# CESNET/GPUJPEG

Hardware: NVIDIA H100
Metric: Mpix/s encode+decode 8k RGB q75 (higher is better)
Workload: dtype f32+i32 (u8 in, i16 coefficients)

## Files before the change

gpujpeg_b200/csrc/gj_encoder.c:

```c
#include <assert.h>
#include <stdlib.h>
#include <string.h>

#include "gj_internal.h"

#define GJ_STRIPES 8
#define GJ_STRIPE_MIN_BYTES ((size_t)8 << 20)

struct gpujpeg_encoder {
    gj_stream_t stream;
    int device;
    struct gpujpeg_parameters param;
    struct gpujpeg_image_parameters param_image;
    int initialised;
    struct gj_geometry geo;
    struct gj_k1_request k1_req;
    struct gj_k1_plan k1;
    uint8_t* d_planes; size_t d_planes_size;
    struct gj_raw_layout raw;
    int quality;
    enum gpujpeg_header_type header_type;
    enum gpujpeg_header_type header_written;
    int flipped;
    unsigned channel_remap;
// ... 434 lines not shown
}

static int fit_huffman_tables(struct gpujpeg_encoder* e)
{
    const struct gj_geometry* g = &e->geo;
    if ( launch_stats(e) || gj_cuda_memcpy_d2h_async(e->h_counts, e->d_counts, GJ_HUFF_COUNTS_BYTES, e->stream) ||
         gj_cuda_stream_sync(e->stream) )
        return -1;
    int used[2] = {0, 0};
    for ( int c = 0; c < g->comp_count; c++ )
        used[g->lay.comp_tbl[c]] = 1;
    for ( int t = 0; t < 2; t++ ) {
        for ( int k = 0; k < 2; k++ ) {
            if ( used[t] ) gj_huff_spec_optimal(e->h_counts + (t * 2 + k) * 256, &e->spec[t][k]);
            else gj_huff_spec_default(t, k, &e->spec[t][k]);
        }
        gj_enc_lut_build(&e->spec[t][0], &e->spec[t][1], &e->h_tab.lut[t]);
    }
    e->spec_custom = 1;
    const size_t need = GJ_HEADER_BASE_CAP + 4 * 256 + gj_exif_tags_bytes(e->extras.exif_tags) + e->extras.com_size;
    if ( need > e->header_cap ) {
        free(e->header);
        e->header = (uint8_t*)malloc(need);
        e->header_cap = e->header ? need : 0;
        if ( !e->header ) return -1;
    }
    e->header_size = gj_write_header(e->header, &e->param, &e->param_image, e->raw_q, e->spec, e->header_type, &e->extras);
    if ( e->header_size + 64 > g->stream_cap ) {
        GJ_ERR("The header (%zu bytes) does not fit the stream buffer of a %dx%d image.\n", e->header_size, g->width, g->height);
        return -1;
    }
    return gj_cuda_memcpy_h2d_async(e->d_tab, &e->h_tab, sizeof e->h_tab, e->stream);
}

static struct gj_k1_request k1_request(const struct gpujpeg_encoder* e, int in)
{
    struct gj_k1_request r;
    memset(&r, 0, sizeof r);
    r.in = in;
    r.libjpeg = e->writer_libjpeg;
    r.flipped = e->flipped != 0;
    r.channel_remap = e->channel_remap != 0;
    r.coef_input = e->coef_input;
    return r;
}

static int reserve_out(struct gpujpeg_encoder* e, size_t size)
{
    if ( e->out_size >= size && e->out_is_pinned == e->out_pinned ) return 0;
    if ( e->out ) {
        if ( e->out_is_pinned ) gj_cuda_free_host(e->out);
        else free(e->out);
    }
    e->out = NULL;
    e->out_size = 0;
    e->out_is_pinned = e->out_pinned;
    if ( e->out_pinned ) {
        if ( gj_cuda_malloc_host((void**)&e->out, size) ) return -1;
    }
    else if ( !(e->out = (uint8_t*)malloc(size)) ) {
        return -1;
    }
    e->out_size = size;
    return 0;
}

static int encoder_init_image(struct gpujpeg_encoder* e, const struct gpujpeg_parameters* p,
                              const struct gpujpeg_image_parameters* pi, const struct gj_k1_request* k1)
{
    gj_geometry_init(&e->geo, p, pi);
    e->geo.stream_cap += e->extras.com_size;
    e->k1_req = *k1;
    gj_k1_choose(&e->geo, k1, &e->k1);
    if ( e->k1.raw_layout && gj_raw_layout_init(&e->raw, pi) ) return -1;
    if ( e->k1.convert && grow((void**)&e->d_planes, &e->d_planes_size, e->k1.planes_bytes) ) return -1;
    const struct gj_geometry* g = &e->geo;
    size_t coef_bytes = g->coef_count * sizeof(int16_t);
    const size_t segblk_all = (size_t)g->seg_mcu * (size_t)g->lay.bpm;
    size_t first_stride = (segblk_all * 48 + 2 + 127) / 128 * 128;
    if ( first_stride > g->slot_stride ) first_stride = g->slot_stride;
    if ( e->slot_stride < first_stride || e->slot_stride > g->slot_stride ) e->slot_stride = first_stride;
    size_t tmp_bytes = (size_t)g->seg_count * e->slot_stride + 256;
    const int segblk = g->seg_mcu * g->lay.bpm;
    size_t spill_bytes = (size_t)g->seg_count * (segblk <= 40 ? segblk : 32) * 32 * sizeof(uint32_t);
    const size_t split_bytes = gj_huffman_split_status_bytes(g->seg_count, segblk, g->slot_stride);
    if ( grow((void**)&e->d_coef, &e->d_coef_size, coef_bytes) ||
         grow((void**)&e->d_nzmask, &e->d_nzmask_size, g->coef_count / 64 * sizeof(uint64_t)) ||
         grow((void**)&e->d_tmp, &e->d_tmp_size, tmp_bytes) ||
         grow((void**)&e->d_spill, &e->d_spill_size, spill_bytes) ||
         grow((void**)&e->d_split, &e->d_split_size, split_bytes) ||
         grow((void**)&e->d_stream, &e->d_stream_size, g->stream_cap + 64) ) {
        GJ_ERR("Encoder device allocation failed (%zu + %zu + %zu bytes): %s\n", coef_bytes, tmp_bytes, g->stream_cap,
               gj_cuda_last_error());
        return -1;
    }
    if ( g->seg_count > e->seg_alloc ) {
        gj_cuda_free(e->d_seg_bytes);
        gj_cuda_free(e->d_seg_off);
        e->d_seg_bytes = NULL;
        e->d_seg_off = NULL;
        e->seg_alloc = 0;
        if ( gj_cuda_malloc((void**)&e->d_seg_bytes, (size_t)g->seg_count * 4) ||
             gj_cuda_malloc((void**)&e->d_seg_off, (size_t)g->seg_count * 8) )
            return -1;
        e->seg_alloc = g->seg_count;
    }
    if ( reserve_out(e, g->stream_cap) ) return -1;
    e->param = *p;
    e->param_image = *pi;
    e->initialised = 1;
    return 0;
}

static int same_image(const struct gpujpeg_image_parameters* a, const struct gpujpeg_image_parameters* b)
{
    return a->width == b->width && a->height == b->height && a->color_space == b->color_space &&
           a->pixel_format == b->pixel_format && a->width_padding == b->width_padding;
}
static gpujpeg_sampling_factor_t packed_sampling(const struct gpujpeg_parameters* p)
{
    gpujpeg_sampling_factor_t r = 0;
    for ( int c = 0; c < p->comp_count && c < 4; c++ )
        r |= (gpujpeg_sampling_factor_t)p->sampling_factor[c].horizontal << (28 - 8 * c) |
             (gpujpeg_sampling_factor_t)p->sampling_factor[c].vertical << (24 - 8 * c);
    return r;
}

static int same_param(const struct gpujpeg_parameters* a, const struct gpujpeg_parameters* b)
{
    if ( a->restart_interval != b->restart_interval || a->interleaved != b->interleaved ||
         a->segment_info != b->segment_info || a->comp_count != b->comp_count ||
         a->color_space_internal != b->color_space_internal )
        return 0;
    for ( int c = 0; c < a->comp_count; c++ )
        if ( a->sampling_factor[c].horizontal != b->sampling_factor[c].horizontal ||
             a->sampling_factor[c].vertical != b->sampling_factor[c].vertical )
            return 0;
    return 1;
}

static struct gpujpeg_parameters adjust_params(struct gpujpeg_encoder* e, const struct gpujpeg_parameters* param,
                                               const struct gpujpeg_image_parameters* pi, int img_changed)
{
    struct gpujpeg_parameters a = *param;
    if ( param->comp_count == 0 ) {
        if ( img_changed || !e->initialised ) {
            const int n = gpujpeg_pixel_format_get_comp_count(pi->pixel_format);
            a.comp_count = n > 3 ? 3 : n;
            struct gj_raw_layout rl;
            const int known = gj_raw_layout_init(&rl, pi) == 0;
            memset(a.sampling_factor, 0, sizeof a.sampling_factor);
            for ( int c = 0; c < a.comp_count; c++ ) {
                a.sampling_factor[c].horizontal = known ? rl.sampling[c].horizontal : 1;
                a.sampling_factor[c].vertical = known ? rl.sampling[c].vertical : 1;
            }
        }
        else {
            a.comp_count = e->param.comp_count;
            memcpy(a.sampling_factor, e->param.sampling_factor, sizeof a.sampling_factor);
        }
    }
    if ( param->restart_interval == RESTART_AUTO ) {
        if ( img_changed || !e->initialised || a.interleaved != e->param.interleaved )
            a.restart_interval =
                gpujpeg_encoder_suggest_restart_interval(pi, packed_sampling(&a), a.interleaved, a.verbose);
        else
            a.restart_interval = e->param.restart_interval;
// ... 582 lines not shown
```

gpujpeg_b200/csrc/gj_huffman.cu:

```cuda
#include <cuda_runtime.h>
#include <stdint.h>

#include "gj_device.cuh"
#include "gj_internal.h"
#include "gj_launch.cuh"

namespace {

constexpr unsigned FULL = 0xFFFFFFFFu;

__device__ __forceinline__ int warp_incl_scan(int v, int lane)
{
#pragma unroll
    for ( int d = 1; d < 32; d <<= 1 ) {
        const int t = __shfl_up_sync(FULL, v, d);
        if ( lane >= d ) v += t;
    }
    return v;
}

__device__ __forceinline__ int scan_of_segment(const gj_scan_layout& L, int g)
{
    return (g >= L.scan_seg_begin[1]) + (g >= L.scan_seg_begin[2]) + (g >= L.scan_seg_begin[3]);
}

__device__ __forceinline__ void segment_block(const gj_scan_layout& L, int scan, int first_mcu, int j, size_t& bi, int& comp,
                                              int& pd)
{
    if ( L.simple ) {
        if ( !L.interleaved ) {
            comp = scan;
            bi = (size_t)L.blk_off[scan] + first_mcu + j;
            pd = 1;
        }
        else {
            const int cps = L.comp_count;
            const int mcu = j / cps;
            comp = j - mcu * cps;
            bi = (size_t)L.blk_off[comp] + first_mcu + mcu;
            pd = cps;
        }
    }
    else if ( !L.interleaved ) {
        comp = scan;
        bi = (size_t)L.blk_off[scan] + first_mcu + j;
        pd = 1;
    }
    else {
        const int mcu = j / L.bpm, i = j - mcu * L.bpm;
        const int m = first_mcu + mcu;
        const int my = m / L.mcu_x, mx = m - my * L.mcu_x;
        comp = L.idx_comp[i];
        bi = (size_t)L.blk_off[comp] + (size_t)(my * L.comp_vs[comp] + L.idx_dy[i]) * L.bcx[comp] + mx * L.comp_hs[comp] +
             L.idx_dx[i];
        pd = L.idx_pred[i];
    }
}


constexpr int HE_WARPS = 8;
constexpr int HE_WORDS = 512;
constexpr int HE_CAP_BITS = (HE_WORDS - 2) * 32;

__device__ __forceinline__ uint32_t flush_words(const uint32_t* buf, int nw, uint8_t* out, uint32_t pos, int lane, uint32_t cap)
{
    for ( int base = 0; base < nw; base += 32 ) {
        const int i = base + lane;
        const uint32_t w = i < nw ? buf[i] : 0u;
        int cnt = 0;
        if ( i < nw ) {
            const uint32_t t = w & (w >> 4) & 0x0F0F0F0Fu;
            const uint32_t ff = t & (t >> 2) & 0x03030303u;
            const uint32_t m = ff & (ff >> 1) & 0x01010101u;
            cnt = 4 + __popc(m);
        }
        const int incl = warp_incl_scan(cnt, lane);
        uint8_t* o = out + pos + (incl - cnt);
        if ( i < nw && pos + (uint32_t)incl <= cap ) {
#pragma unroll
            for ( int j = 3; j >= 0; j-- ) {
                const uint8_t b = (uint8_t)(w >> (8 * j));
                *o++ = b;
                if ( b == 0xFF ) *o++ = 0;
            }
        }
        pos += (uint32_t)__shfl_sync(FULL, incl, 31);
    }
    return pos;
}

constexpr int HE_PRIV = 25;
constexpr int HE_SPILL = 32;
constexpr int HE_HEAD = 12;
template <class Put>
__device__ __forceinline__ int code_block(int dc, int pred, uint64_t nz, const int16_t* head16, const int16_t* __restrict__ blk,
                                          const uint32_t (*s_ac)[256], const uint32_t (*s_dc)[16], int tbl, Put put)
{
    uint64_t acc = 0;
    int nb = 0, wi = 0;
    auto emit = [&](int len, uint32_t bits) {
        acc = (acc << len) | (uint64_t)bits;
        nb += len;
        if ( nb >= 32 ) {
            put(wi, (uint32_t)(acc >> (nb - 32)));
            wi++;
            nb -= 32;
        }
    };
    const int diff = dc - pred;
    const int dcat = gj_category(diff);
    const uint32_t de = s_dc[tbl][dcat];
    emit((int)(de & 31u) + dcat, ((de >> 5) << dcat) | (dcat ? gj_value_bits(diff, dcat) : 0u));
    uint32_t mlo = (uint32_t)nz & ~1u, mhi = (uint32_t)(nz >> 32);
    int last = 0;
    const uint32_t zrl = s_ac[tbl][0xF0];
    while ( mlo | mhi ) {
        int k;
        if ( mlo ) { k = __ffs((int)mlo) - 1; mlo &= mlo - 1; }
        else { k = 32 + __ffs((int)mhi) - 1; mhi &= mhi - 1; }
        int run = k - last - 1;
        last = k;
        const int v = k < 16 ? (int)head16[k] : (int)__ldg(blk + k);
        const int size = gj_category(v);
        while ( run > 15 ) {
            emit((int)(zrl & 31u), zrl >> 5);
            run -= 16;
        }
        const uint32_t e = s_ac[tbl][(run << 4) | size];
        emit((int)(e & 31u) + size, ((e >> 5) << size) | gj_value_bits(v, size));
    }
    if ( last < 63 ) {
        const uint32_t e = s_ac[tbl][0];
        emit((int)(e & 31u), e >> 5);
    }
    if ( nb ) put(wi, (uint32_t)(acc << (32 - nb)));
    return 32 * wi + nb;
}

constexpr int HE_SMEM = (2 * 256 + 2 * 16 + HE_WARPS * HE_WORDS + HE_WARPS * 32 * HE_PRIV + HE_WARPS * 32 * HE_HEAD) * 4;

__global__ void __launch_bounds__(HE_WARPS * 32)
k_huff_encode(const int16_t* __restrict__ coef, const uint64_t* __restrict__ nzmask, const __grid_constant__ gj_scan_layout lay,
              int seg_mcu, int seg_count, uint8_t* __restrict__ tmp, size_t slot_stride,
              uint32_t* __restrict__ seg_bytes, uint32_t* __restrict__ spill_all, const gj_dev_enc_tables* __restrict__ tables,
              uint64_t* __restrict__ info, unsigned long long* __restrict__ place_status, int n_status)
{
    gj_pdl_wait();
    if ( threadIdx.x == 0 && (int)blockIdx.x < n_status ) place_status[blockIdx.x] = 0ull;
    const uint32_t slot_cap = (uint32_t)slot_stride;
    extern __shared__ __align__(16) uint32_t he_smem[];
    uint32_t (*s_ac)[256] = reinterpret_cast<uint32_t (*)[256]>(he_smem);
    uint32_t (*s_dc)[16] = reinterpret_cast<uint32_t (*)[16]>(he_smem + 512);
    uint32_t* s_buf = he_smem + 512 + 32;
    uint32_t* s_priv = s_buf + HE_WARPS * HE_WORDS;
    uint32_t* s_head = s_priv + HE_WARPS * 32 * HE_PRIV;

    for ( int i = threadIdx.x; i < 512; i += blockDim.x )
        s_ac[i >> 8][i & 255] = tables->lut[i >> 8].ac[i & 255];
    if ( threadIdx.x < 32 ) s_dc[threadIdx.x >> 4][threadIdx.x & 15] = tables->lut[threadIdx.x >> 4].dc[threadIdx.x & 15];
    __syncthreads();

    const int warp = threadIdx.x >> 5, lane = threadIdx.x & 31;
    const int g = blockIdx.x * HE_WARPS + warp;
    if ( g >= seg_count ) return;
    const int scan = scan_of_segment(lay, g), s = g - lay.scan_seg_begin[scan];
    const int first_mcu = s * seg_mcu;
    const int mcus = min(seg_mcu, lay.scan_mcus[scan] - first_mcu);
    const int nblocks = mcus * lay.bpm;
    uint32_t* buf = s_buf + warp * HE_WORDS;
    uint32_t* priv = s_priv + (warp * 32 + lane) * HE_PRIV;
    uint32_t* spill = spill_all + ((size_t)g * 32 + lane) * HE_SPILL;
    uint32_t* head = s_head + (warp * 32 + lane) * HE_HEAD;
    const int16_t* head16 = reinterpret_cast<const int16_t*>(head);
    uint8_t* out = tmp + (size_t)g * slot_stride;
    uint32_t out_pos = 0;
    int carry = 0;

    for ( int i = lane; i < HE_WORDS; i += 32 )
        buf[i] = 0;
    __syncwarp();

    int dc_before = 0;
    uint64_t nz_next = 0;
    uint4 ha_next = make_uint4(0u, 0u, 0u, 0u), hb_next = ha_next;
    size_t bi_next = 0;
    int comp_next = 0, pd_next = 1;
    {
        const int j = lane;
        if ( j < nblocks ) {
            segment_block(lay, scan, first_mcu, j, bi_next, comp_next, pd_next);
            nz_next = __ldg(nzmask + bi_next);
            ha_next = __ldg(reinterpret_cast<const uint4*>(coef + bi_next * 64));
            hb_next = __ldg(reinterpret_cast<const uint4*>(coef + bi_next * 64) + 1);
        }
    }
    for ( int base = 0; base < nblocks; base += 32 ) {
        const int j = base + lane;
        const bool active = j < nblocks;
        const int comp = comp_next, pd = pd_next;
        const int tbl = lay.comp_tbl[comp];
        const int16_t* blk = coef + bi_next * 64;

        const uint64_t nz = nz_next;
        const int dc = (int)(short)(ha_next.x & 0xFFFFu);
        reinterpret_cast<uint4*>(head)[0] = ha_next;
        reinterpret_cast<uint4*>(head)[1] = hb_next;
        nz_next = 0;
        ha_next = hb_next = make_uint4(0u, 0u, 0u, 0u);
        {
            const int jn = j + 32;
            if ( jn < nblocks ) {
                segment_block(lay, scan, first_mcu, jn, bi_next, comp_next, pd_next);
                nz_next = __ldg(nzmask + bi_next);
                ha_next = __ldg(reinterpret_cast<const uint4*>(coef + bi_next * 64));
                hb_next = __ldg(reinterpret_cast<const uint4*>(coef + bi_next * 64) + 1);
            }
        }
        const int from = (lane - pd) & 31;
        int pred = __shfl_sync(FULL, dc, from);
        const int pred_before = __shfl_sync(FULL, dc_before, from);
        if ( lane < pd ) pred = pred_before;
        if ( j < pd ) pred = 0;
        dc_before = dc;

        int len = 0;
        if ( active ) {
            len = code_block(dc, pred, nz, head16, blk, s_ac, s_dc, tbl, [&](int wi, uint32_t w) {
                if ( wi < HE_PRIV ) priv[wi] = w;
                else spill[wi - HE_PRIV] = w;
            });
        }
        const int incl = warp_incl_scan(len, lane);
        const int excl = incl - len;

        int lane0 = 0;
        while ( lane0 < 32 ) {
            const int rel0 = __shfl_sync(FULL, excl, lane0);
            const int mypos = carry + (excl - rel0);
            const bool fits = lane >= lane0 && mypos + len <= HE_CAP_BITS;
            const int nfit = __popc(__ballot_sync(FULL, fits));
            if ( nfit == 0 ) break;
            const bool mine = lane >= lane0 && lane < lane0 + nfit;
            if ( mine && len > 0 ) {
                const int nw = (len + 31) >> 5;
                const int d0 = mypos >> 5, sh = mypos & 31;
                const int endbit = mypos + len;
                uint32_t prev = 0;
                for ( int q = 0; q <= nw; q++ ) {
                    const uint32_t w = q < nw ? (q < HE_PRIV ? priv[q] : spill[q - HE_PRIV]) : 0u;
                    const uint32_t o = sh ? (prev | (w >> sh)) : w;
                    prev = sh ? (w << (32 - sh)) : 0u;
                    const int d = d0 + q;
                    if ( 32 * d >= endbit ) break;
                    if ( 32 * d >= mypos && 32 * d + 32 <= endbit ) buf[d] = o;
                    else atomicOr(&buf[d], o);
                }
            }
            __syncwarp();
            const int lastl = lane0 + nfit - 1;
            const int newbits = carry + (__shfl_sync(FULL, incl, lastl) - rel0);
            const int nwords = newbits >> 5;
            out_pos = flush_words(buf, nwords, out, out_pos, lane, slot_cap);
            __syncwarp();
            const uint32_t tail = buf[nwords];
            __syncwarp();
            for ( int i = lane; i <= nwords; i += 32 )
                buf[i] = 0;
            __syncwarp();
            if ( lane == 0 ) buf[0] = tail;
            __syncwarp();
            carry = newbits & 31;
            lane0 += nfit;
        }
    }

    if ( lane == 0 ) {
        uint32_t w = buf[0];
        const int nbytes = (carry + 7) >> 3;
        if ( carry & 7 ) w |= ((1u << (8 - (carry & 7))) - 1u) << (32 - nbytes * 8);
        uint32_t n = out_pos;
        for ( int q = 0; q < nbytes; q++ ) {
            const uint8_t b = (uint8_t)(w >> (24 - 8 * q));
            if ( n + 2u <= slot_cap ) {
                out[n] = b;
                if ( b == 0xFF ) out[n + 1] = 0;
            }
            n += b == 0xFF ? 2u : 1u;
        }
        seg_bytes[g] = n;
        if ( n + 2u > slot_cap ) {
            atomicOr(reinterpret_cast<unsigned long long*>(info + 1), 2ull);
            atomicMax(reinterpret_cast<unsigned long long*>(info + 2), (unsigned long long)n + 2ull);
        }
    }
}

constexpr int HP_MAXBLK = 40;
constexpr int HP_THREADS_MAX = HE_WARPS * HP_MAXBLK;
static_assert(HE_WARPS * HE_WORDS >= HP_THREADS_MAX * HE_HEAD, "heads must fit into the stream buffers");
constexpr int HP_SMEM = (2 * 256 + 2 * 16 + HE_WARPS * HE_WORDS + HE_WARPS * HP_MAXBLK * HE_PRIV + HE_WARPS * HP_MAXBLK) * 4;

struct SegPick {
    int n[GJ_MAX_COMP], lo[GJ_MAX_COMP];
    int total;
    int zero_status;
};
__device__ __forceinline__ int pick_segment(const SegPick& P, int j)
{
#pragma unroll
    for ( int k = 0; k < GJ_MAX_COMP; k++ ) {
        if ( j < P.n[k] ) return P.lo[k] + j;
        j -= P.n[k];
    }
    return P.lo[0];
}

__global__ void __launch_bounds__(HP_THREADS_MAX)
k_huff_encode_packed(const int16_t* __restrict__ coef, const uint64_t* __restrict__ nzmask,
                     const __grid_constant__ gj_scan_layout lay, int seg_mcu, const __grid_constant__ SegPick pick,
                     uint8_t* __restrict__ tmp, size_t slot_stride, uint32_t* __restrict__ seg_bytes,
                     uint32_t* __restrict__ spill_all, const gj_dev_enc_tables* __restrict__ tables, uint64_t* __restrict__ info,
                     unsigned long long* __restrict__ place_status, int n_status)
{
    gj_pdl_wait();
    if ( pick.zero_status )
        for ( int i = blockIdx.x * blockDim.x + threadIdx.x; i < n_status; i += gridDim.x * blockDim.x )
            place_status[i] = 0ull;
    const uint32_t slot_cap = (uint32_t)slot_stride;
    extern __shared__ __align__(16) uint32_t he_smem[];
    uint32_t (*s_ac)[256] = reinterpret_cast<uint32_t (*)[256]>(he_smem);
    uint32_t (*s_dc)[16] = reinterpret_cast<uint32_t (*)[16]>(he_smem + 512);
    uint32_t* s_buf = he_smem + 512 + 32;
    uint32_t* s_priv = s_buf + HE_WARPS * HE_WORDS;
    uint32_t* s_head = s_buf;
    uint32_t* s_len = s_priv + HE_WARPS * HP_MAXBLK * HE_PRIV;

    for ( int i = threadIdx.x; i < 512; i += blockDim.x )
        s_ac[i >> 8][i & 255] = tables->lut[i >> 8].ac[i & 255];
    if ( threadIdx.x < 32 ) s_dc[threadIdx.x >> 4][threadIdx.x & 15] = tables->lut[threadIdx.x >> 4].dc[threadIdx.x & 15];
    __syncthreads();

    const int warp = threadIdx.x >> 5, lane = threadIdx.x & 31;
    const int g0 = blockIdx.x * HE_WARPS;
    const int segblk = seg_mcu * lay.bpm;

    {
        uint32_t* head = s_head + threadIdx.x * HE_HEAD;
        const int16_t* head16 = reinterpret_cast<const int16_t*>(head);
        for ( int lb = threadIdx.x; lb < HE_WARPS * segblk; lb += blockDim.x ) {
            const int sl = lb / segblk, j = lb - sl * segblk;
            if ( g0 + sl >= pick.total ) break;
            const int g = pick_segment(pick, g0 + sl);
            const int scan = scan_of_segment(lay, g), s = g - lay.scan_seg_begin[scan];
            const int first_mcu = s * seg_mcu;
            const int nblocks = min(seg_mcu, lay.scan_mcus[scan] - first_mcu) * lay.bpm;
            if ( j >= nblocks ) continue;
            size_t bi;
            int comp, pd;
            segment_block(lay, scan, first_mcu, j, bi, comp, pd);
            const int tbl = lay.comp_tbl[comp];
            const int16_t* blk = coef + bi * 64;
            const uint64_t nz = __ldg(nzmask + bi);
            const uint4 ha = __ldg(reinterpret_cast<const uint4*>(blk)), hb = __ldg(reinterpret_cast<const uint4*>(blk) + 1);
            int pred = 0;
            if ( j >= pd ) {
                size_t bp;
                int cp, pp;
                segment_block(lay, scan, first_mcu, j - pd, bp, cp, pp);
                pred = __ldg(coef + bp * 64);
            }
            reinterpret_cast<uint4*>(head)[0] = ha;
            reinterpret_cast<uint4*>(head)[1] = hb;
            const int dc = (int)(short)(ha.x & 0xFFFFu);
            uint32_t* priv = s_priv + lb * HE_PRIV;
            uint32_t* spill = spill_all + ((size_t)g * segblk + j) * HE_SPILL;
            s_len[lb] = (uint32_t)code_block(dc, pred, nz, head16, blk, s_ac, s_dc, tbl, [&](int wi, uint32_t w) {
                if ( wi < HE_PRIV ) priv[wi] = w;
                else spill[wi - HE_PRIV] = w;
            });
        }
    }
    __syncthreads();

    if ( warp >= HE_WARPS || g0 + warp >= pick.total ) return;
    const int g = pick_segment(pick, g0 + warp);
    const int scan = scan_of_segment(lay, g), s = g - lay.scan_seg_begin[scan];
    const int nblocks = min(seg_mcu, lay.scan_mcus[scan] - s * seg_mcu) * lay.bpm;
    uint32_t* buf = s_buf + warp * HE_WORDS;
    uint8_t* out = tmp + (size_t)g * slot_stride;
    uint32_t out_pos = 0;
    int carry = 0;
    for ( int i = lane; i < HE_WORDS; i += 32 )
        buf[i] = 0;
    __syncwarp();
    auto place = [&](const uint32_t* priv, const uint32_t* spill, int mypos, int len) {
        const int nw = (len + 31) >> 5;
        const int d0 = mypos >> 5, sh = mypos & 31;
        const int endbit = mypos + len;
        uint32_t prev = 0;
        for ( int q = 0; q <= nw; q++ ) {
            const uint32_t w = q < nw ? (q < HE_PRIV ? priv[q] : spill[q - HE_PRIV]) : 0u;
            const uint32_t o = sh ? (prev | (w >> sh)) : w;
            prev = sh ? (w << (32 - sh)) : 0u;
            const int d = d0 + q;
            if ( 32 * d >= endbit ) break;
            if ( 32 * d >= mypos && 32 * d + 32 <= endbit ) buf[d] = o;
            else atomicOr(&buf[d], o);
        }
    };
    {
        const int j0 = lane, j1 = lane + 32;
        const int len0 = j0 < nblocks ? (int)s_len[warp * segblk + j0] : 0;
        const int len1 = j1 < nblocks ? (int)s_len[warp * segblk + j1] : 0;
        const int incl0 = warp_incl_scan(len0, lane);
        const int total0 = __shfl_sync(FULL, incl0, 31);
        const int incl1 = warp_incl_scan(len1, lane);
        const int total = total0 + __shfl_sync(FULL, incl1, 31);
        if ( total <= HE_CAP_BITS ) {
            if ( len0 > 0 )
                place(s_priv + (warp * segblk + j0) * HE_PRIV, spill_all + ((size_t)g * segblk + j0) * HE_SPILL, incl0 - len0, len0);
            if ( len1 > 0 )
                place(s_priv + (warp * segblk + j1) * HE_PRIV, spill_all + ((size_t)g * segblk + j1) * HE_SPILL,
                      total0 + incl1 - len1, len1);
            __syncwarp();
            const int nwords = total >> 5;
            out_pos = flush_words(buf, nwords, out, out_pos, lane, slot_cap);
            __syncwarp();
            carry = total & 31;
            if ( lane == 0 ) buf[0] = buf[nwords];
            __syncwarp();
        }
        else {
            for ( int base = 0; base < nblocks; base += 32 ) {
                const int j = base + lane;
                const bool active = j < nblocks;
                const int len = active ? (int)s_len[warp * segblk + j] : 0;
                const uint32_t* priv = s_priv + (warp * segblk + (active ? j : 0)) * HE_PRIV;
                const uint32_t* spill = spill_all + ((size_t)g * segblk + (active ? j : 0)) * HE_SPILL;
                const int incl = warp_incl_scan(len, lane);
                const int excl = incl - len;
                int lane0 = 0;
                while ( lane0 < 32 ) {
                    const int rel0 = __shfl_sync(FULL, excl, lane0);
                    const int mypos = carry + (excl - rel0);
                    const bool fits = lane >= lane0 && mypos + len <= HE_CAP_BITS;
                    const int nfit = __popc(__ballot_sync(FULL, fits));
                    if ( nfit == 0 ) break;
                    const bool mine = lane >= lane0 && lane < lane0 + nfit;
                    if ( mine && len > 0 ) place(priv, spill, mypos, len);
                    __syncwarp();
                    const int lastl = lane0 + nfit - 1;
                    const int newbits = carry + (__shfl_sync(FULL, incl, lastl) - rel0);
                    const int nwords = newbits >> 5;
                    out_pos = flush_words(buf, nwords, out, out_pos, lane, slot_cap);
                    __syncwarp();
                    const uint32_t tail = buf[nwords];
                    __syncwarp();
                    for ( int i = lane; i <= nwords; i += 32 )
                        buf[i] = 0;
                    __syncwarp();
                    if ( lane == 0 ) buf[0] = tail;
                    __syncwarp();
                    carry = newbits & 31;
                    lane0 += nfit;
                }
            }
        }
    }
    if ( lane == 0 ) {
        uint32_t w = buf[0];
        const int nbytes = (carry + 7) >> 3;
        if ( carry & 7 ) w |= ((1u << (8 - (carry & 7))) - 1u) << (32 - nbytes * 8);
        uint32_t n = out_pos;
        for ( int q = 0; q < nbytes; q++ ) {
            const uint8_t b = (uint8_t)(w >> (24 - 8 * q));
            if ( n + 2u <= slot_cap ) {
                out[n] = b;
                if ( b == 0xFF ) out[n + 1] = 0;
            }
            n += b == 0xFF ? 2u : 1u;
        }
        seg_bytes[g] = n;
        if ( n + 2u > slot_cap ) {
            atomicOr(reinterpret_cast<unsigned long long*>(info + 1), 2ull);
            atomicMax(reinterpret_cast<unsigned long long*>(info + 2), (unsigned long long)n + 2ull);
        }
    }
}

struct ScanSegs {
    int begin[GJ_MAX_COMP + 1];
};
struct ScanPrefix {
    int len[GJ_MAX_COMP], off[GJ_MAX_COMP];
};
__device__ __forceinline__ int scan_of_segment(const ScanSegs& S, int g)
{
    return (g >= S.begin[1]) + (g >= S.begin[2]) + (g >= S.begin[3]);
}

#ifndef GJ_CP_LANES
#define GJ_CP_LANES 8
#endif
constexpr int CP_LANES = GJ_CP_LANES;
constexpr int CP_SEGS = 256 / CP_LANES;
#define PL_VALID (1ull << 62)
#define PL_VALUE ((1ull << 62) - 1ull)
__global__ void __launch_bounds__(256)
k_huff_place(const uint8_t* __restrict__ tmp, size_t slot_stride, const uint32_t* __restrict__ seg_bytes, int seg_count,
             const __grid_constant__ ScanSegs segs, const uint8_t* __restrict__ sos, const __grid_constant__ ScanPrefix pre,
             uint32_t header_size, uint64_t stream_cap, uint8_t* __restrict__ stream,
             volatile unsigned long long* status , uint64_t* __restrict__ seg_pos ,
             uint64_t* __restrict__ info, uint64_t* __restrict__ info_next )
{
    gj_pdl_wait();
    __shared__ uint32_t s_excl[CP_SEGS];
    __shared__ unsigned long long s_part[8];
    __shared__ uint32_t s_own;
    const int lane = threadIdx.x & 31, warp = threadIdx.x >> 5;
    const int tile = blockIdx.x;
    const int sl = threadIdx.x & (CP_LANES - 1), ls = threadIdx.x / CP_LANES;
// ... 116 lines not shown

template <class Prev>
__device__ __forceinline__ uint64_t hs_look_back(volatile unsigned long long* status, long long j, Prev prev)
{
    uint64_t sum = 0;
    while ( j >= 0 ) {
        unsigned long long v;
        do {
            v = status[j];
        } while ( v == 0ull );
        sum += v & HS_VALUE;
        if ( v & HS_INC ) break;
        j = prev(j);
    }
    return sum;
}

__device__ __forceinline__ int hs_cta_excl_scan(int v, int& total, int* s_warp)
{
    const int lane = threadIdx.x & 31, warp = threadIdx.x >> 5, nwarps = blockDim.x >> 5;
    const int incl = warp_incl_scan(v, lane);
    if ( lane == 31 ) s_warp[warp] = incl;
    __syncthreads();
    int before = 0;
    total = 0;
    for ( int w = 0; w < nwarps; w++ ) {
        const int t = s_warp[w];
        if ( w < warp ) before += t;
        total += t;
    }
    return before + incl - v;
}

__device__ __forceinline__ int hs_segment(const gj_scan_layout& L, int seg_mcu, int g, int& scan, int& s)
{
    scan = scan_of_segment(L, g);
    s = g - L.scan_seg_begin[scan];
    return min(seg_mcu, L.scan_mcus[scan] - s * seg_mcu) * L.bpm;
}

__global__ void __launch_bounds__(GJ_HS_CHUNK)
k_huff_chunk(const int16_t* __restrict__ coef, const uint64_t* __restrict__ nzmask, const __grid_constant__ gj_scan_layout lay,
             int seg_mcu, int nch, uint8_t* __restrict__ tmp, size_t slot_stride, const gj_dev_enc_tables* __restrict__ tables,
             uint64_t* __restrict__ info, volatile unsigned long long* chunk_status)
{
    gj_pdl_wait();
    extern __shared__ __align__(16) uint32_t hc_smem[];
    uint32_t (*s_ac)[256] = reinterpret_cast<uint32_t (*)[256]>(hc_smem);
    uint32_t (*s_dc)[16] = reinterpret_cast<uint32_t (*)[16]>(hc_smem + 512);
    uint32_t* s_priv = hc_smem + 512 + 32;
    uint32_t* s_head = s_priv + GJ_HS_CHUNK * HC_PRIV + 4;
    int* s_warp = reinterpret_cast<int*>(s_head + GJ_HS_CHUNK * HE_HEAD);

    const int g = blockIdx.x / nch, c = blockIdx.x - g * nch;
    int scan, s;
    const int nblocks = hs_segment(lay, seg_mcu, g, scan, s);
    const int j0 = c * GJ_HS_CHUNK;
    if ( j0 >= nblocks ) return;
    for ( int i = threadIdx.x; i < 512; i += blockDim.x )
        s_ac[i >> 8][i & 255] = tables->lut[i >> 8].ac[i & 255];
    if ( threadIdx.x < 32 ) s_dc[threadIdx.x >> 4][threadIdx.x & 15] = tables->lut[threadIdx.x >> 4].dc[threadIdx.x & 15];
    __syncthreads();

    const int first_mcu = s * seg_mcu, j = j0 + (int)threadIdx.x;
    uint32_t* priv = s_priv + threadIdx.x * HC_PRIV;
    int len = 0;
    if ( j < nblocks ) {
        size_t bi;
        int comp, pd;
        segment_block(lay, scan, first_mcu, j, bi, comp, pd);
        uint32_t* head = s_head + threadIdx.x * HE_HEAD;
        const int16_t* blk = coef + bi * 64;
        const uint64_t nz = __ldg(nzmask + bi);
        const uint4 ha = __ldg(reinterpret_cast<const uint4*>(blk)), hb = __ldg(reinterpret_cast<const uint4*>(blk) + 1);
        int pred = 0;
        if ( j >= pd ) {
            size_t bp;
            int cp, pp;
            segment_block(lay, scan, first_mcu, j - pd, bp, cp, pp);
            pred = __ldg(coef + bp * 64);
        }
        reinterpret_cast<uint4*>(head)[0] = ha;
        reinterpret_cast<uint4*>(head)[1] = hb;
        len = code_block((int)(short)(ha.x & 0xFFFFu), pred, nz, reinterpret_cast<const int16_t*>(head), blk, s_ac, s_dc,
                         lay.comp_tbl[comp], [&](int wi, uint32_t w) { priv[wi] = w; });
    }
    int total;
    const int excl = hs_cta_excl_scan(len, total, s_warp);

    const long long me = blockIdx.x;
    if ( threadIdx.x == 0 ) {
        unsigned long long before = 0;
        if ( c == 0 ) chunk_status[me] = HS_INC | (unsigned long long)total;
        else {
            chunk_status[me] = HS_AGG | (unsigned long long)total;
            before = hs_look_back(chunk_status, me - 1, [&](long long q) { return q - 1 > (long long)g * nch - 1 ? q - 1 : -1ll; });
            chunk_status[me] = HS_INC | (before + (unsigned long long)total);
        }
    }

    const int segblk = seg_mcu * lay.bpm;
    const uint32_t share = (uint32_t)(slot_stride / 4 / (size_t)segblk);
    const int nblk = min(GJ_HS_CHUNK, nblocks - j0);
    const uint32_t nw = ((uint32_t)total + 31u) >> 5;
    if ( nw > (uint32_t)nblk * share ) {
        if ( threadIdx.x == 0 ) {
            atomicOr(reinterpret_cast<unsigned long long*>(info + 1), 2ull);
            const unsigned long long need = (unsigned long long)((nw + nblk - 1) / nblk) * 4ull * (unsigned long long)segblk;
            atomicMax(reinterpret_cast<unsigned long long*>(info + 2), need);
        }
        return;
    }
    uint32_t* area = reinterpret_cast<uint32_t*>(tmp + (size_t)g * slot_stride) + (size_t)j0 * share;
    if ( len ) {
        area[excl >> 5] = 0u;
        area[(excl + len - 1) >> 5] = 0u;
    }
    __syncthreads();
    if ( len ) {
        const int nwb = (len + 31) >> 5;
        const int d0 = excl >> 5, sh = excl & 31, endbit = excl + len;
        uint32_t prev = 0;
        for ( int q = 0; q <= nwb; q++ ) {
            const uint32_t w = q < nwb ? priv[q] : 0u;
            const uint32_t o = sh ? (prev | (w >> sh)) : w;
            prev = sh ? (w << (32 - sh)) : 0u;
            const int d = d0 + q;
            if ( 32 * d >= endbit ) break;
            if ( 32 * d >= excl && 32 * d + 32 <= endbit ) area[d] = o;
            else atomicOr(&area[d], o);
        }
    }
}

__global__ void __launch_bounds__(HT_THREADS)
k_huff_stuff(const uint8_t* __restrict__ tmp, size_t slot_stride, const __grid_constant__ gj_scan_layout lay, int seg_mcu, int nch,
             int tps, const unsigned long long* __restrict__ chunk_status, const uint8_t* __restrict__ sos,
             const __grid_constant__ ScanPrefix pre, uint32_t header_size, uint64_t stream_cap, uint8_t* __restrict__ stream,
             volatile unsigned long long* tile_status, uint64_t* __restrict__ seg_pos, uint64_t* __restrict__ info,
             uint64_t* __restrict__ info_next)
{
    gj_pdl_wait();
    __shared__ __align__(16) uint8_t s_out[2 * GJ_HS_TILE];
    __shared__ unsigned long long s_end[HT_MAXCH];
    __shared__ int s_warp[HT_THREADS / 32];
    __shared__ unsigned long long s_base;
    const int seg_count = lay.scan_seg_begin[GJ_MAX_COMP];
    if ( info[1] & 2ull ) {
        if ( blockIdx.x == 0 && threadIdx.x == 0 && info_next ) info_next[0] = info_next[1] = info_next[2] = info_next[3] = 0ull;
        return;
    }
    const int g = (int)(blockIdx.x / (unsigned)tps);
    const long long i = (long long)blockIdx.x - (long long)g * tps;
    int scan, s;
    const int nblocks = hs_segment(lay, seg_mcu, g, scan, s);
    const int nch_g = gj_hs_chunks(nblocks);
    const unsigned long long* E = chunk_status + (size_t)g * nch;
    const uint64_t bits = E[nch_g - 1] & HS_VALUE;
    const long long ntiles = (long long)gj_hs_tiles(bits);
    if ( i >= ntiles ) return;
    const uint64_t nbytes = gj_hs_seg_bytes(bits);
    const uint64_t P0 = (uint64_t)i * GJ_HS_TILE * 8;
    const uint32_t tile_bytes = (uint32_t)min((uint64_t)GJ_HS_TILE, nbytes - (uint64_t)i * GJ_HS_TILE);

    int lo = 0, hi = nch_g - 1;
    while ( lo < hi ) {
        const int step = (hi - lo + HT_THREADS - 1) / HT_THREADS;
        const int c = lo + (int)threadIdx.x * step;
// ... 789 lines not shown
```

gpujpeg_b200/csrc/gj_internal.h:

```cpp
#ifndef GJ_INTERNAL_H
#define GJ_INTERNAL_H

#include <stddef.h>
#include <stdint.h>
#include <stdio.h>

#include "../../include/gpujpeg_b200.h"

#ifdef __cplusplus
extern "C" {
#endif

#define GJ_MAX_COMP 4
#define GJ_SOS_LEN_1 10

#define GJ_ERR(...) (void)(fprintf(stderr, "[GPUJPEG] [Error] " __VA_ARGS__))
#define GJ_WARN(...) (void)(fprintf(stderr, "[GPUJPEG] [Warning] " __VA_ARGS__))
#define GJ_VERBOSE(v, ...) do { if ( (v) >= GPUJPEG_LL_VERBOSE ) (void)fprintf(stderr, "[GPUJPEG] [Verbose] " __VA_ARGS__); } while ( 0 )
#define GJ_DEBUG(v, ...) do { if ( (v) >= GPUJPEG_LL_DEBUG ) (void)fprintf(stderr, "[GPUJPEG] [Debug] " __VA_ARGS__); } while ( 0 )

extern const uint8_t gj_zigzag_to_natural[64];
extern const uint8_t gj_natural_to_zigzag[64];

struct gj_huff_spec {
    uint8_t bits[17];
    uint8_t vals[256];
    int nvals;
};
void gj_huff_spec_default(int cls , int kind , struct gj_huff_spec* spec);
void gj_huff_spec_optimal(const uint64_t freq[256], struct gj_huff_spec* spec);

void gj_quant_raw(int cls, int quality, uint8_t raw_zz[64]);
void gj_quant_forward_zz(const uint8_t raw_zz[64], float fwd_zz[64]);

struct gj_enc_lut {
    uint32_t ac[256];
    uint32_t dc[16];
};
void gj_enc_lut_build(const struct gj_huff_spec* dc, const struct gj_huff_spec* ac, struct gj_enc_lut* lut);

#define GJ_DEC_LOOK_BITS 9
struct gj_dec_lut {
    uint16_t look[1 << GJ_DEC_LOOK_BITS];
    uint32_t maxcode[18];
    int32_t valoff[18];
    uint8_t vals[256];
};
int gj_dec_lut_build(const struct gj_huff_spec* spec, struct gj_dec_lut* lut);

#define GJ_DEC_FAST_BITS 10
#define GJ_DEC_FAST_SUBS 8
#define GJ_DEC_FAST_TOTAL_SHIFT 7
#define GJ_DEC_FAST_TOTAL_MASK (31u << GJ_DEC_FAST_TOTAL_SHIFT)
#define GJ_DEC_FAST_SIZE_SHIFT 16
struct gj_dec_fast {
    uint32_t e[1 << GJ_DEC_FAST_BITS];
    uint32_t sub[GJ_DEC_FAST_SUBS][1 << (16 - GJ_DEC_FAST_BITS)];
};
void gj_dec_fast_build(const struct gj_huff_spec* spec, int is_ac, struct gj_dec_fast* fast);

#define GJ_MAX_MCU_BLOCKS 10

struct gj_comp_geo {
    int hs, vs;
    int width, height;
    int bcx, bcy;
    int nblk;
    int blk_off;
};

struct gj_scan_layout {
    int simple;
    int interleaved;
    int comp_count;
    int scan_count;
    int bpm;
    int mcu_x;
    int blk_off[GJ_MAX_COMP];
    int bcx[GJ_MAX_COMP];
    int scan_seg_begin[GJ_MAX_COMP + 1];
    int scan_mcus[GJ_MAX_COMP];
    uint8_t idx_comp[GJ_MAX_MCU_BLOCKS], idx_dx[GJ_MAX_MCU_BLOCKS], idx_dy[GJ_MAX_MCU_BLOCKS], idx_pred[GJ_MAX_MCU_BLOCKS];
    uint8_t comp_hs[GJ_MAX_COMP], comp_vs[GJ_MAX_COMP];
    uint8_t comp_tbl[GJ_MAX_COMP];
};

struct gj_geometry {
    int width, height, comp_count;
    int pitch;
    int data_width, data_height;
    int bcx, bcy, nblk;
    int interleaved;
    int restart_interval;
    int seg_mcu;
    int scan_count;
    int comps_per_scan;
// ... 472 lines not shown
```

profiles/k2_times.py:

```python
import os, sys
ROOT = os.path.dirname(os.path.dirname(os.path.abspath(__file__)))
sys.path.insert(0, ROOT); sys.path.insert(0, os.path.join(ROOT, "tests"))
import torch
import _oracle as o
import gpujpeg_b200 as g
size = sys.argv[1] if len(sys.argv) > 1 else "8k"
kind = sys.argv[2] if len(sys.argv) > 2 else "photo"
w, h, rst = {"8k": (7680, 4320, 36), "4k": (3840, 2160, 24), "hd": (1920, 1080, 24)}[size]
d_raw = torch.from_numpy(o.gen_image(kind, w, h)).cuda()
enc = g.Encoder(stream=torch.cuda.current_stream().cuda_stream)
ref = enc.encode(d_raw, 75, rst, 0)
def timeit(fn, n=20):
    for _ in range(3): fn()
    torch.cuda.synchronize()
    e0, e1 = torch.cuda.Event(enable_timing=True), torch.cuda.Event(enable_timing=True)
    e0.record()
    for _ in range(n): fn()
    e1.record(); torch.cuda.synchronize()
    return e0.elapsed_time(e1) / n * 1e3
print(size, kind, "K1 %.1f us  K2 %.1f us  K1+K2 %.1f us  (jpeg %d B)" % (timeit(lambda: enc.run_resident(d_raw, 1)), timeit(lambda: enc.run_resident(d_raw, 2)),
                                                                     timeit(lambda: enc.run_resident(d_raw, 3)), ref.size))
import numpy as np
assert np.array_equal(enc.encode(d_raw, 75, rst, 0), ref)
```

Baseline: 60620.

## Stage per-block coefficients via cp.async into swizzled smem slots in parallel Huffman

```diff
diff --git a/gpujpeg_b200/csrc/gj_encoder.c b/gpujpeg_b200/csrc/gj_encoder.c
--- a/gpujpeg_b200/csrc/gj_encoder.c
+++ b/gpujpeg_b200/csrc/gj_encoder.c
@@ -540,7 +540,7 @@
     if ( e->slot_stride < first_stride || e->slot_stride > g->slot_stride ) e->slot_stride = first_stride;
     size_t tmp_bytes = (size_t)g->seg_count * e->slot_stride + 256;
     const int segblk = g->seg_mcu * g->lay.bpm;
-    size_t spill_bytes = (size_t)g->seg_count * (segblk <= 40 ? segblk : 32) * 32 * sizeof(uint32_t);
+    size_t spill_bytes = (size_t)g->seg_count * (segblk <= 40 ? (size_t)segblk * GJ_HP_SPILL : 32 * 32) * sizeof(uint32_t);
     const size_t split_bytes = gj_huffman_split_status_bytes(g->seg_count, segblk, g->slot_stride);
     if ( grow((void**)&e->d_coef, &e->d_coef_size, coef_bytes) ||
          grow((void**)&e->d_nzmask, &e->d_nzmask_size, g->coef_count / 64 * sizeof(uint64_t)) ||
diff --git a/gpujpeg_b200/csrc/gj_huffman.cu b/gpujpeg_b200/csrc/gj_huffman.cu
--- a/gpujpeg_b200/csrc/gj_huffman.cu
+++ b/gpujpeg_b200/csrc/gj_huffman.cu
@@ -92,9 +92,20 @@
 constexpr int HE_PRIV = 25;
 constexpr int HE_SPILL = 32;
 constexpr int HE_HEAD = 12;
-template <class Put>
-__device__ __forceinline__ int code_block(int dc, int pred, uint64_t nz, const int16_t* head16, const int16_t* __restrict__ blk,
-                                          const uint32_t (*s_ac)[256], const uint32_t (*s_dc)[16], int tbl, Put put)
+struct HeadThenGlobal {
+    const int16_t* head16;
+    const int16_t* blk;
+    __device__ __forceinline__ int operator()(int k) const { return k < 16 ? (int)head16[k] : (int)__ldg(blk + k); }
+};
+struct StagedBlock {
+    const int16_t* slot;
+    int swz;
+    __device__ __forceinline__ int operator()(int k) const { return (int)slot[(((k >> 3) ^ swz) << 3) | (k & 7)]; }
+};
+
+template <class Coef, class Put>
+__device__ __forceinline__ int code_block(int dc, int pred, uint64_t nz, Coef ac, const uint32_t (*s_ac)[256],
+                                          const uint32_t (*s_dc)[16], int tbl, Put put)
 {
     uint64_t acc = 0;
     int nb = 0, wi = 0;
@@ -120,7 +131,7 @@
         else { k = 32 + __ffs((int)mhi) - 1; mhi &= mhi - 1; }
         int run = k - last - 1;
         last = k;
-        const int v = k < 16 ? (int)head16[k] : (int)__ldg(blk + k);
+        const int v = ac(k);
         const int size = gj_category(v);
         while ( run > 15 ) {
             emit((int)(zrl & 31u), zrl >> 5);
@@ -225,7 +236,7 @@
 
         int len = 0;
         if ( active ) {
-            len = code_block(dc, pred, nz, head16, blk, s_ac, s_dc, tbl, [&](int wi, uint32_t w) {
+            len = code_block(dc, pred, nz, HeadThenGlobal{head16, blk}, s_ac, s_dc, tbl, [&](int wi, uint32_t w) {
                 if ( wi < HE_PRIV ) priv[wi] = w;
                 else spill[wi - HE_PRIV] = w;
             });
@@ -297,8 +308,20 @@
 
 constexpr int HP_MAXBLK = 40;
 constexpr int HP_THREADS_MAX = HE_WARPS * HP_MAXBLK;
-static_assert(HE_WARPS * HE_WORDS >= HP_THREADS_MAX * HE_HEAD, "heads must fit into the stream buffers");
-constexpr int HP_SMEM = (2 * 256 + 2 * 16 + HE_WARPS * HE_WORDS + HE_WARPS * HP_MAXBLK * HE_PRIV + HE_WARPS * HP_MAXBLK) * 4;
+constexpr int HP_PRIV = 9;
+static_assert(HP_PRIV + GJ_HP_SPILL >= 54, "an 8x8 block can need 54 words (64 x (16-bit code + 11 value bits))");
+constexpr int HP_SLOT = 32;
+constexpr int HP_STAGE = HP_THREADS_MAX * HP_SLOT;
+static_assert(HP_STAGE >= HE_WARPS * HE_WORDS, "the stream buffers must fit into the block slots' area");
+constexpr int HP_SMEM = (2 * 256 + 2 * 16 + HP_STAGE + HE_WARPS * HP_MAXBLK * HP_PRIV + HE_WARPS * HP_MAXBLK) * 4;
+static_assert((2 * 256 + 2 * 16) % 4 == 0, "the block slots must be 16-byte aligned (cp.async)");
+static_assert(4 * (HP_SMEM + 1024) <= 228 * 1024, "4 CTAs per SM (1 KB reserved per CTA, 228 KB per SM on sm_90)");
+
+__device__ __forceinline__ void cp_async16(void* dst, const void* src)
+{
+    asm volatile("cp.async.cg.shared.global [%0], [%1], 16;" ::"r"((uint32_t)__cvta_generic_to_shared(dst)), "l"(src) : "memory");
+}
+__device__ __forceinline__ void cp_async_wait_all() { asm volatile("cp.async.wait_all;" ::: "memory"); }
 
 struct SegPick {
     int n[GJ_MAX_COMP], lo[GJ_MAX_COMP];
@@ -331,9 +354,9 @@
     uint32_t (*s_ac)[256] = reinterpret_cast<uint32_t (*)[256]>(he_smem);
     uint32_t (*s_dc)[16] = reinterpret_cast<uint32_t (*)[16]>(he_smem + 512);
     uint32_t* s_buf = he_smem + 512 + 32;
-    uint32_t* s_priv = s_buf + HE_WARPS * HE_WORDS;
-    uint32_t* s_head = s_buf;
-    uint32_t* s_len = s_priv + HE_WARPS * HP_MAXBLK * HE_PRIV;
+    uint32_t* s_slot = s_buf;
+    uint32_t* s_priv = s_buf + HP_STAGE;
+    uint32_t* s_len = s_priv + HE_WARPS * HP_MAXBLK * HP_PRIV;
 
     for ( int i = threadIdx.x; i < 512; i += blockDim.x )
         s_ac[i >> 8][i & 255] = tables->lut[i >> 8].ac[i & 255];
@@ -345,8 +368,6 @@
     const int segblk = seg_mcu * lay.bpm;
 
     {
-        uint32_t* head = s_head + threadIdx.x * HE_HEAD;
-        const int16_t* head16 = reinterpret_cast<const int16_t*>(head);
         for ( int lb = threadIdx.x; lb < HE_WARPS * segblk; lb += blockDim.x ) {
             const int sl = lb / segblk, j = lb - sl * segblk;
             if ( g0 + sl >= pick.total ) break;
@@ -360,8 +381,11 @@
             segment_block(lay, scan, first_mcu, j, bi, comp, pd);
             const int tbl = lay.comp_tbl[comp];
             const int16_t* blk = coef + bi * 64;
+            uint32_t* slot = s_slot + lb * HP_SLOT;
+            const int swz = lb & 7;
             const uint64_t nz = __ldg(nzmask + bi);
-            const uint4 ha = __ldg(reinterpret_cast<const uint4*>(blk)), hb = __ldg(reinterpret_cast<const uint4*>(blk) + 1);
+            cp_async16(slot + 4 * (0 ^ swz), blk);
+            cp_async16(slot + 4 * (1 ^ swz), blk + 8);
             int pred = 0;
             if ( j >= pd ) {
                 size_t bp;
@@ -369,14 +393,18 @@
                 segment_block(lay, scan, first_mcu, j - pd, bp, cp, pp);
                 pred = __ldg(coef + bp * 64);
             }
-            reinterpret_cast<uint4*>(head)[0] = ha;
-            reinterpret_cast<uint4*>(head)[1] = hb;
-            const int dc = (int)(short)(ha.x & 0xFFFFu);
-            uint32_t* priv = s_priv + lb * HE_PRIV;
-            uint32_t* spill = spill_all + ((size_t)g * segblk + j) * HE_SPILL;
-            s_len[lb] = (uint32_t)code_block(dc, pred, nz, head16, blk, s_ac, s_dc, tbl, [&](int wi, uint32_t w) {
-                if ( wi < HE_PRIV ) priv[wi] = w;
-                else spill[wi - HE_PRIV] = w;
+            const int live = gj_coef_live_chunks(nz);
+#pragma unroll
+            for ( int c = 2; c < 8; c++ )
+                if ( c < live ) cp_async16(slot + 4 * (c ^ swz), blk + 8 * c);
+            cp_async_wait_all();
+            const StagedBlock ac{reinterpret_cast<const int16_t*>(slot), swz};
+            const int dc = ac(0);
+            uint32_t* priv = s_priv + lb * HP_PRIV;
+            uint32_t* spill = spill_all + ((size_t)g * segblk + j) * GJ_HP_SPILL;
+            s_len[lb] = (uint32_t)code_block(dc, pred, nz, ac, s_ac, s_dc, tbl, [&](int wi, uint32_t w) {
+                if ( wi < HP_PRIV ) priv[wi] = w;
+                else spill[wi - HP_PRIV] = w;
             });
         }
     }
@@ -399,7 +427,7 @@
         const int endbit = mypos + len;
         uint32_t prev = 0;
         for ( int q = 0; q <= nw; q++ ) {
-            const uint32_t w = q < nw ? (q < HE_PRIV ? priv[q] : spill[q - HE_PRIV]) : 0u;
+            const uint32_t w = q < nw ? (q < HP_PRIV ? priv[q] : spill[q - HP_PRIV]) : 0u;
             const uint32_t o = sh ? (prev | (w >> sh)) : w;
             prev = sh ? (w << (32 - sh)) : 0u;
             const int d = d0 + q;
@@ -418,9 +446,9 @@
         const int total = total0 + __shfl_sync(FULL, incl1, 31);
         if ( total <= HE_CAP_BITS ) {
             if ( len0 > 0 )
-                place(s_priv + (warp * segblk + j0) * HE_PRIV, spill_all + ((size_t)g * segblk + j0) * HE_SPILL, incl0 - len0, len0);
+                place(s_priv + (warp * segblk + j0) * HP_PRIV, spill_all + ((size_t)g * segblk + j0) * GJ_HP_SPILL, incl0 - len0, len0);
             if ( len1 > 0 )
-                place(s_priv + (warp * segblk + j1) * HE_PRIV, spill_all + ((size_t)g * segblk + j1) * HE_SPILL,
+                place(s_priv + (warp * segblk + j1) * HP_PRIV, spill_all + ((size_t)g * segblk + j1) * GJ_HP_SPILL,
                       total0 + incl1 - len1, len1);
             __syncwarp();
             const int nwords = total >> 5;
@@ -435,8 +463,8 @@
                 const int j = base + lane;
                 const bool active = j < nblocks;
                 const int len = active ? (int)s_len[warp * segblk + j] : 0;
-                const uint32_t* priv = s_priv + (warp * segblk + (active ? j : 0)) * HE_PRIV;
-                const uint32_t* spill = spill_all + ((size_t)g * segblk + (active ? j : 0)) * HE_SPILL;
+                const uint32_t* priv = s_priv + (warp * segblk + (active ? j : 0)) * HP_PRIV;
+                const uint32_t* spill = spill_all + ((size_t)g * segblk + (active ? j : 0)) * GJ_HP_SPILL;
                 const int incl = warp_incl_scan(len, lane);
                 const int excl = incl - len;
                 int lane0 = 0;
@@ -719,8 +747,8 @@
         }
         reinterpret_cast<uint4*>(head)[0] = ha;
         reinterpret_cast<uint4*>(head)[1] = hb;
-        len = code_block((int)(short)(ha.x & 0xFFFFu), pred, nz, reinterpret_cast<const int16_t*>(head), blk, s_ac, s_dc,
-                         lay.comp_tbl[comp], [&](int wi, uint32_t w) { priv[wi] = w; });
+        len = code_block((int)(short)(ha.x & 0xFFFFu), pred, nz, HeadThenGlobal{reinterpret_cast<const int16_t*>(head), blk}, s_ac,
+                         s_dc, lay.comp_tbl[comp], [&](int wi, uint32_t w) { priv[wi] = w; });
     }
     int total;
     const int excl = hs_cta_excl_scan(len, total, s_warp);
diff --git a/gpujpeg_b200/csrc/gj_internal.h b/gpujpeg_b200/csrc/gj_internal.h
--- a/gpujpeg_b200/csrc/gj_internal.h
+++ b/gpujpeg_b200/csrc/gj_internal.h
@@ -12,6 +12,7 @@
 #endif
 
 #define GJ_MAX_COMP 4
+#define GJ_HP_SPILL 45
 #define GJ_SOS_LEN_1 10
 
 #define GJ_ERR(...) (void)(fprintf(stderr, "[GPUJPEG] [Error] " __VA_ARGS__))
diff --git a/profiles/k2_times.py b/profiles/k2_times.py
--- a/profiles/k2_times.py
+++ b/profiles/k2_times.py
@@ -1,24 +1,98 @@
-import os, sys
-ROOT = os.path.dirname(os.path.dirname(os.path.abspath(__file__)))
-sys.path.insert(0, ROOT); sys.path.insert(0, os.path.join(ROOT, "tests"))
-import torch
-import _oracle as o
-import gpujpeg_b200 as g
-size = sys.argv[1] if len(sys.argv) > 1 else "8k"
-kind = sys.argv[2] if len(sys.argv) > 2 else "photo"
-w, h, rst = {"8k": (7680, 4320, 36), "4k": (3840, 2160, 24), "hd": (1920, 1080, 24)}[size]
-d_raw = torch.from_numpy(o.gen_image(kind, w, h)).cuda()
-enc = g.Encoder(stream=torch.cuda.current_stream().cuda_stream)
-ref = enc.encode(d_raw, 75, rst, 0)
-def timeit(fn, n=20):
-    for _ in range(3): fn()
-    torch.cuda.synchronize()
-    e0, e1 = torch.cuda.Event(enable_timing=True), torch.cuda.Event(enable_timing=True)
-    e0.record()
-    for _ in range(n): fn()
-    e1.record(); torch.cuda.synchronize()
-    return e0.elapsed_time(e1) / n * 1e3
-print(size, kind, "K1 %.1f us  K2 %.1f us  K1+K2 %.1f us  (jpeg %d B)" % (timeit(lambda: enc.run_resident(d_raw, 1)), timeit(lambda: enc.run_resident(d_raw, 2)),
-                                                                     timeit(lambda: enc.run_resident(d_raw, 3)), ref.size))
-import numpy as np
-assert np.array_equal(enc.encode(d_raw, 75, rst, 0), ref)
+import argparse
+import hashlib
+import json
+import os
+import subprocess
+import sys
+
+HERE = os.path.dirname(os.path.abspath(__file__))
+CASES = [("8k", "photo", "4:4:4", 0), ("8k", "random", "4:4:4", 0), ("8k", "photo", "4:2:0", 1), ("4k", "photo", "4:4:4", 0),
+         ("hd", "photo", "4:4:4", 0)]
+SIZES = {"8k": (7680, 4320, 36), "4k": (3840, 2160, 24), "hd": (1920, 1080, 24)}
+
+
+def sm_clock():
+    q = subprocess.run(["nvidia-smi", "-i", "0", "--query-gpu=clocks.sm", "--format=csv,noheader,nounits"], capture_output=True,
+                       text=True)
+    return q.stdout.strip()
+
+
+def worker(root, launches):
+    sys.path[:0] = [root, os.path.join(root, "tests")]
+    import numpy as np
+    import torch
+    import _oracle as o
+    import gpujpeg_b200 as g
+    dev = torch.device("cuda", 0)
+    stream = torch.cuda.current_stream().cuda_stream
+
+    def median_us(fn):
+        for _ in range(10):
+            fn()
+        ev = [(torch.cuda.Event(enable_timing=True), torch.cuda.Event(enable_timing=True)) for _ in range(launches)]
+        for e0, e1 in ev:
+            e0.record()
+            fn()
+            e1.record()
+        torch.cuda.synchronize()
+        return float(np.median([e0.elapsed_time(e1) * 1e3 for e0, e1 in ev]))
+
+    def batch_us(fn):
+        for _ in range(10):
+            fn()
+        e0, e1 = torch.cuda.Event(enable_timing=True), torch.cuda.Event(enable_timing=True)
+        e0.record()
+        for _ in range(launches):
+            fn()
+        e1.record()
+        torch.cuda.synchronize()
+        return e0.elapsed_time(e1) * 1e3 / launches
+
+    out = {"tree": root}
+    for size, kind, ss, il in CASES:
+        w, h, rst = SIZES[size]
+        if il:
+            rst = 6
+        d_raw = torch.from_numpy(o.gen_image(kind, w, h)).to(dev)
+        enc, dec = g.Encoder(stream=stream, pinned_output=True), g.Decoder(stream=stream)
+        jpeg = enc.encode(d_raw, 75, rst, il, subsampling=ss)
+        d_out = torch.empty((h, w, 3), dtype=torch.uint8, device=dev)
+        dec.decode(jpeg, out=d_out)
+        torch.cuda.synchronize()
+
+        def step():
+            enc.run_resident(d_raw, 3)
+            dec.run_resident(d_out, 7)
+
+        name = "%s_%s_%s" % (size, kind, ss.replace(":", ""))
+        out["k2_us_" + name] = round(median_us(lambda: enc.run_resident(d_raw, 2)), 2)
+        out["step_us_" + name] = round(batch_us(step), 2)
+        out["sm_mhz_" + name] = sm_clock()
+        last = enc.stream()
+        out["jpeg_" + name] = hashlib.sha256(last.tobytes()).hexdigest()[:16]
+        assert np.array_equal(last, jpeg), "the timed K2 produced other bytes than the first call"
+        enc.close()
+        dec.close()
+    print(json.dumps(out), flush=True)
+
+
+def main():
+    ap = argparse.ArgumentParser()
+    ap.add_argument("--trees", nargs="*", default=["."])
+    ap.add_argument("--rounds", type=int, default=3)
+    ap.add_argument("--launches", type=int, default=60)
+    ap.add_argument("--worker", default=None)
+    a = ap.parse_args()
+    if a.worker:
+        return worker(a.worker, a.launches)
+    q = subprocess.run(["nvidia-smi", "--query-gpu=name,power.limit,clocks.max.sm", "--format=csv,noheader"],
+                       capture_output=True, text=True)
+    print(json.dumps({"gpu": q.stdout.strip()}), flush=True)
+    for _ in range(a.rounds):
+        for t in a.trees:
+            subprocess.run([sys.executable, os.path.abspath(__file__), "--worker", os.path.abspath(t), "--launches",
+                            str(a.launches)], check=True)
+
+
+if __name__ == "__main__":
+    main()
```

Result: faster. 62870 (median of 6 runs) (+3.7%).
